# GSByeon/multi-speaker-tacotron-tensorflow

Hardware: AMD Instinct MI355X
Metric: mel-frames/sec (batched decode) (higher is better)
Workload: dtype f32 storage and accumulation; feed-forward GEMMs as 3-term split-bf16 MFMA (bf16x3), the attention memory layer as 6-term split-bf16 MFMA (operands split three ways: fp32-grade); recurrent / decoder mat-vecs exact fp32

## Files before the change

multi-speaker-tacotron-tensorflow_amd/csrc/taco_bigru_xcd.h:

```cpp
#pragma once
#include "taco_decoder_xcd.h"

#define GX_H 256
#define GX_BLK 16
typedef __attribute__((address_space(3))) float gx_lds_float;
__device__ __forceinline__ void gx_load_lds16(const float* gsrc, unsigned lds_dst) {
  unsigned keep;
  asm volatile("s_mov_b32 %0, m0\n\ts_mov_b32 m0, %2\n\ts_nop 0\n\tglobal_load_lds_dwordx4 %1, off\n\ts_mov_b32 m0, %0"
               : "=&s"(keep) : "v"(gsrc), "s"(lds_dst) : "memory");
}

#define GD_MEMBERS 32
#define GD_NREG 24
__host__ __device__ inline size_t gd_ring_floats(int RG) { return (size_t)2 * 2 * GX_BLK * RG * 24; }
__host__ __device__ inline size_t gd_lds_floats(int RG) { return gd_ring_floats(RG) + (size_t)4 * RG * GX_H + 64; }
__host__ __device__ constexpr size_t gd_xbuf_granules(int RG) { return (size_t)DX_NGROUP * 4 * RG * GX_H; }

template <int RG, int NT>
struct GdPoll {
  static constexpr int NI = (RG * GX_H + NT - 1) / NT;
  unsigned long long g[NI];
};
template <int RG, int NT>
__device__ __forceinline__ void gd_request(const dx_gu64* X, int tid, GdPoll<RG, NT>& p) {
// ... 326 lines not shown
    xs[i] = 0.f;
  }
  constexpr int QPG = UPM / 4, NIT = 2 * GX_BLK * 3 * QPG, NLD = (NIT + NT - 1) / NT;
  static_assert(NIT % 64 == 0, "a wave's 64 items are all inside the block or all outside");
  const unsigned xq_lds = (unsigned)(size_t)(gx_lds_float*)xq;
  auto blk_fetch = [&](int s0, int ring) {
#pragma unroll
    for (int u = 0; u < NLD; ++u) {
      if (u * NT + wave * 64 < NIT) {
        const int i = u * NT + tid;
        const int c = i % QPG, g = (i / QPG) % 3, j = (i / (3 * QPG)) % GX_BLK, d = i / (3 * QPG * GX_BLK);
        const int sx = min(s0 + j, T - 1);
        const float* src = a.xproj + ((size_t)row * T + sx) * 6 * H + d * 3 * H + g * H + member * UPM + 4 * c;
        const unsigned dst = __builtin_amdgcn_readfirstlane(xq_lds + (unsigned)(ring * SLOT + 4 * (u * NT + wave * 64)) * 4u);
        gx_load_lds16(src, dst);
      }
    }
  };
  blk_fetch(0, 0);
  blk_fetch(GX_BLK, 1);
  asm volatile("s_waitcnt vmcnt(0)" ::: "memory");
  __syncthreads();

  const int ui_outer = lane / LPU;
  float x0[2][3], hv[2], gv[2];
#pragma unroll
  for (int d = 0; d < 2; ++d) { hv[d] = hs[d * H + member * UPM + wave * UPW + ui_outer]; gv[d] = 0.f; }
  unsigned long long pre = 0ull, pre2 = 0ull;

  const int tid_outer = tid, lane_outer = lane;
  for (int s = 0; s < T; ++s) {
    const unsigned tag = (unsigned)s + 1u;
    int tid = tid_outer, lane = lane_outer;
    asm volatile("" : "+v"(tid), "+v"(lane));
    const int ui = lane / LPU, unit = member * UPM + wave * UPW + ui;
    const bool pub = (lane & (LPU - 1)) == 0;
    const bool active = s < L;
    GO_STAMP(0);
    const int sb = s & (GX_BLK - 1), ring = (s / GX_BLK) & 1;
    if (sb == 0 && s > 0) blk_fetch(s + GX_BLK, ring ^ 1);
    auto request = [&](const dx_gu64* Xv, int D) {
      if ((wave >> 2) == D) pre = __hip_atomic_load(Xv + (tid & 255), __ATOMIC_RELAXED, __HIP_MEMORY_SCOPE_AGENT);
    };
    auto request2 = [&](const dx_gu64* Xv, int D) {
      if ((wave >> 2) == D) pre2 = __hip_atomic_load(Xv + (tid & 255), __ATOMIC_RELAXED, __HIP_MEMORY_SCOPE_AGENT);
    };
    int csite = 0;
    auto collect = [&](const dx_gu64* Xv, unsigned tg, float* dst, int D) {
      if ((wave >> 2) == D) {
        float v[1];
        if ((unsigned)(pre2 >> 32) == tg) v[0] = __uint_as_float((unsigned)pre2);
        else if ((unsigned)(pre >> 32) == tg) v[0] = __uint_as_float((unsigned)pre);
        else { go_knob_sleep(GO_KNOB(8 + csite)); dx_poll<1>(Xv + (tid & 255), 0, tg, v, rt); }
        dst[tid & 255] = v[0];
      }
    };
    auto gates = [&](auto Dc, const dx_gu64* Xn, int Dn) {
      constexpr int D = decltype(Dc)::value;
      constexpr int R0 = (NREG / 2) * D;
#pragma unroll
      for (int g = 0; g < 3; ++g) x0[D][g] = xq[(size_t)ring * SLOT + ((size_t)(D * GX_BLK + sb) * 3 + g) * UPM + wave * UPW + ui];
      const float4 hx = *reinterpret_cast<const float4*>(hs + D * H + 4 * lane);
      taco_f32x2 acc[UPW];
#pragma unroll
      for (int i = 0; i < UPW; ++i) acc[i] = (taco_f32x2){W[R0 + 8 * i] * hx.x, W[R0 + 8 * i + 4] * hx.x};
#pragma unroll
      for (int i = 0; i < UPW; ++i) acc[i] = __builtin_elementwise_fma((taco_f32x2){hx.y, hx.y}, (taco_f32x2){W[R0 + 8 * i + 1], W[R0 + 8 * i + 5]}, acc[i]);
#pragma unroll
      for (int i = 0; i < UPW; ++i) acc[i] = __builtin_elementwise_fma((taco_f32x2){hx.z, hx.z}, (taco_f32x2){W[R0 + 8 * i + 2], W[R0 + 8 * i + 6]}, acc[i]);
#pragma unroll
      for (int i = 0; i < UPW; ++i) acc[i] = __builtin_elementwise_fma((taco_f32x2){hx.w, hx.w}, (taco_f32x2){W[R0 + 8 * i + 3], W[R0 + 8 * i + 7]}, acc[i]);
      if (GO_REQ2 && Xn && GO_KNOB(D) == 0) request2(Xn, Dn);
      else if (GO_KNOB(D) == 2) pre2 = 0ull;
      float v[2 * UPW], sm[2];
#pragma unroll
      for (int i = 0; i < UPW; ++i) { v[2 * i] = acc[i].x; v[2 * i + 1] = acc[i].y; }
      go_reduce<UPW, 2>(v, sm);
      if (GO_REQ2 && Xn && GO_KNOB(D) == 1) request2(Xn, Dn);
      const float rr = dx_sigmoid_fast(sm[0] + x0[D][0]);
      gv[D] = dx_sigmoid_fast(sm[1] + x0[D][1]);
      float rh = rr * hv[D];
      asm volatile("" : "+v"(pre), "+v"(pre2), "+v"(rh));
      if (pub) { if (GO_DYN) dx_publish(X + (size_t)D * 2 * H + unit, rh, tag, rt); else go_publish<WT>(X + (size_t)D * 2 * H + unit, rh, tag); }
      if (TAPE && pub && active) {
        float* gs = a.gsave + ((size_t)row * T + (D ? L - 1 - s : s)) * 6 * H + D * 3 * H + unit;
        gs[0] = rr; gs[H] = gv[D];
      }
    };
    auto cand = [&](auto Dc, const dx_gu64* Xn, int Dn) {
      constexpr int D = decltype(Dc)::value;
      constexpr int R0 = (NREG / 2) * D + 8 * UPW;
      const float4 hx = *reinterpret_cast<const float4*>(xs + D * H + 4 * lane);
      float v[UPW], sm[1];
      if constexpr (UPW >= 2) {
        taco_f32x2 acc[UPW / 2];
#pragma unroll
        for (int i = 0; i < UPW / 2; ++i) acc[i] = (taco_f32x2){W[R0 + 8 * i] * hx.x, W[R0 + 8 * i + 4] * hx.x};
#pragma unroll
        for (int i = 0; i < UPW / 2; ++i) acc[i] = __builtin_elementwise_fma((taco_f32x2){hx.y, hx.y}, (taco_f32x2){W[R0 + 8 * i + 1], W[R0 + 8 * i + 5]}, acc[i]);
#pragma unroll
        for (int i = 0; i < UPW / 2; ++i) acc[i] = __builtin_elementwise_fma((taco_f32x2){hx.z, hx.z}, (taco_f32x2){W[R0 + 8 * i + 2], W[R0 + 8 * i + 6]}, acc[i]);
#pragma unroll
        for (int i = 0; i < UPW / 2; ++i) acc[i] = __builtin_elementwise_fma((taco_f32x2){hx.w, hx.w}, (taco_f32x2){W[R0 + 8 * i + 3], W[R0 + 8 * i + 7]}, acc[i]);
#pragma unroll
        for (int i = 0; i < UPW / 2; ++i) { v[2 * i] = acc[i].x; v[2 * i + 1] = acc[i].y; }
      } else {
        taco_f32x2 acc = (taco_f32x2){W[R0] * hx.x, W[R0 + 1] * hx.y};
        acc = __builtin_elementwise_fma((taco_f32x2){hx.z, hx.w}, (taco_f32x2){W[R0 + 2], W[R0 + 3]}, acc);
        v[0] = acc.x + acc.y;
      }
      if (GO_REQ2 && Xn && GO_KNOB(2 + D) == 0) request2(Xn, Dn);
      else if (GO_KNOB(2 + D) == 2) pre2 = 0ull;
      go_reduce<UPW, 1>(v, sm);
      if (GO_REQ2 && Xn && GO_KNOB(2 + D) == 1) request2(Xn, Dn);
      const float cc = taco_tanh_fast(sm[0] + x0[D][2]);
      float blend = gv[D] * hv[D] + (1.f - gv[D]) * cc;
      DX_PIN(blend);
      float nv = active ? blend : hv[D];
      asm volatile("" : "+v"(pre), "+v"(pre2), "+v"(nv));
      if (pub) {
        if (GO_DYN) dx_publish(X + (size_t)(D * 2 + 1) * H + unit, nv, tag, rt); else go_publish<WT>(X + (size_t)(D * 2 + 1) * H + unit, nv, tag);
        const int t = (D && active) ? (L - 1 - s) : s;
        a.out[((size_t)row * T + t) * 2 * H + D * H + unit] = active ? nv : 0.f;
        if (TAPE && active) a.gsave[((size_t)row * T + t) * 6 * H + D * 3 * H + 2 * H + unit] = cc;
      }
      hv[D] = nv;
    };
    using F = std::integral_constant<int, 0>;
    using Bk = std::integral_constant<int, 1>;
    const dx_gu64* X_rhF = X;                  const dx_gu64* X_hF = X + (size_t)H;
    const dx_gu64* X_rhB = X + (size_t)2 * H;  const dx_gu64* X_hB = X + (size_t)3 * H;
    gates(F{}, s > 0 ? X_hB : nullptr, 1);
    GO_STAMP(1);
    csite = 0;
    if (s > 0) collect(X_hB, tag - 1u, hs + H, 1);
    __syncthreads();
    GO_STAMP(2);
    go_knob_sleep(GO_KNOB(4 + 1));
    request(X_rhF, 0);
    gates(Bk{}, X_rhF, 0);
    GO_STAMP(3);
    csite = 1;
    collect(X_rhF, tag, xs, 0);
    __syncthreads();
    GO_STAMP(4);
    go_knob_sleep(GO_KNOB(4 + 2));
    request(X_rhB, 1);
    cand(F{}, X_rhB, 1);
    GO_STAMP(5);
    csite = 2;
    collect(X_rhB, tag, xs + H, 1);
    __syncthreads();
    GO_STAMP(6);
    go_knob_sleep(GO_KNOB(4 + 3));
    request(X_hF, 0);
    cand(Bk{}, X_hF, 0);
    GO_STAMP(7);
    csite = 3;
    collect(X_hF, tag, hs, 0);
    if (sb == GX_BLK - 1) asm volatile("s_waitcnt vmcnt(0)" ::: "memory");
    __syncthreads();
    GO_STAMP(8);
    go_knob_sleep(GO_KNOB(4 + 0));
    request(X_hB, 1);
  }
}
// ... 485 lines not shown
```

multi-speaker-tacotron-tensorflow_amd/csrc/taco_decoder_xcd.h:

```cpp
#pragma once
#include "taco_kernels.h"

typedef __attribute__((address_space(1))) unsigned long long dx_gu64;
typedef __attribute__((address_space(1))) unsigned dx_gu32;

#define DX_NT 512
#define DX_NW 8
#define DX_GROUP 32
#define DX_NGROUP 8
#define DX_W 256
#define DX_P2 128
#define DX_P3 64
#define DX_SPIN_LIMIT (1u << 21)
#ifndef DX_POLL_SLEEP
#define DX_POLL_SLEEP 0
#endif
#ifndef DX_FIRST_POLL_DELAY
#define DX_FIRST_POLL_DELAY 5
#endif
#ifndef DX_PRIO_OLD
#define DX_PRIO_OLD 1
#endif
#ifndef DX_POLL_DELAY_B
#define DX_POLL_DELAY_B 5
// ... 266 lines not shown
  for (int r0 = 0; r0 < RG; r0 += 4) {
    if constexpr (RG >= 4) asm volatile("" : "+v"(xv[r0]), "+v"(xv[r0 + 1]), "+v"(xv[r0 + 2]), "+v"(xv[r0 + 3]));
    else if constexpr (RG == 2) asm volatile("" : "+v"(xv[0]), "+v"(xv[1]));
  }
}
#define DXQ_FMA(acc, xs, wp) \
  do { if (DX_DIET) acc = __builtin_elementwise_fma((taco_f32x2){xs, xs}, wp, acc); else { acc.x = fmaf((wp).x, xs, acc.x); acc.y = fmaf((wp).y, xs, acc.y); } } while (0)
template <int RG>
__device__ __forceinline__ void dxq_zero(taco_f32x2 (&acc)[RG]) {
#pragma unroll
  for (int r = 0; r < RG; ++r) acc[r] = (taco_f32x2){0.f, 0.f};
}
template <int REG0, int RG, int LD = DXS_LD>
__device__ __forceinline__ void dxw_single(const taco_f32x2 (&WP)[DX_NWP], const float* x, int lane, float (&acc)[1][RG]) {
  constexpr int k = REG0 / 2;
  dx_f32x4 xr[RG];
  dx_rows4<RG, LD>(x, lane, xr);
#pragma unroll
  for (int r = 0; r < RG; ++r) {
    const dx_f32x4 xv = xr[r];
    acc[0][r] = fmaf(WP[k].x, xv.x, acc[0][r]); acc[0][r] = fmaf(WP[k].y, xv.y, acc[0][r]);
    acc[0][r] = fmaf(WP[k + 1].x, xv.z, acc[0][r]); acc[0][r] = fmaf(WP[k + 1].y, xv.w, acc[0][r]);
  }
}
template <int REG0, int RG, int LD = DXS_LD>
__device__ __forceinline__ void dxw_pair(const taco_f32x2 (&WP)[DX_NWP], const float* x, int lane, taco_f32x2 (&acc)[RG]) {
  constexpr int k = REG0 / 2;
  dx_f32x4 xr[RG];
  dx_rows4<RG, LD>(x, lane, xr);
#pragma unroll
  for (int r = 0; r < RG; ++r) {
    const dx_f32x4 xv = xr[r];
    DXQ_FMA(acc[r], xv.x, WP[k]); DXQ_FMA(acc[r], xv.y, WP[k + 1]); DXQ_FMA(acc[r], xv.z, WP[k + 2]); DXQ_FMA(acc[r], xv.w, WP[k + 3]);
  }
}
template <int REG0, int RG, int LD = DXS_LD>
__device__ __forceinline__ void dxw_quad(const taco_f32x2 (&WP)[DX_NWP], const float* x, int lane, taco_f32x2 (&p0)[RG], taco_f32x2 (&p1)[RG]) {
  constexpr int k = REG0 / 2;
  dx_f32x4 xr[RG];
  dx_rows4<RG, LD>(x, lane, xr);
#pragma unroll
  for (int r = 0; r < RG; ++r) {
    const dx_f32x4 xv = xr[r];
    DXQ_FMA(p0[r], xv.x, WP[k]); DXQ_FMA(p1[r], xv.x, WP[k + 4]);
    DXQ_FMA(p0[r], xv.y, WP[k + 1]); DXQ_FMA(p1[r], xv.y, WP[k + 5]);
    DXQ_FMA(p0[r], xv.z, WP[k + 2]); DXQ_FMA(p1[r], xv.z, WP[k + 6]);
    DXQ_FMA(p0[r], xv.w, WP[k + 3]); DXQ_FMA(p1[r], xv.w, WP[k + 7]);
  }
}
template <int REGP, int REGS, int RG, int LD = DXS_LD>
__device__ __forceinline__ void dxw_pair_single(const taco_f32x2 (&WP)[DX_NWP], const float* x, int lane, taco_f32x2 (&p)[RG], float (&sg)[1][RG]) {
  constexpr int k = REGP / 2, ks = REGS / 2;
  dx_f32x4 xr[RG];
  dx_rows4<RG, LD>(x, lane, xr);
#pragma unroll
  for (int r = 0; r < RG; ++r) {
    const dx_f32x4 xv = xr[r];
    DXQ_FMA(p[r], xv.x, WP[k]); sg[0][r] = fmaf(WP[ks].x, xv.x, sg[0][r]);
    DXQ_FMA(p[r], xv.y, WP[k + 1]); sg[0][r] = fmaf(WP[ks].y, xv.y, sg[0][r]);
    DXQ_FMA(p[r], xv.z, WP[k + 2]); sg[0][r] = fmaf(WP[ks + 1].x, xv.z, sg[0][r]);
    DXQ_FMA(p[r], xv.w, WP[k + 3]); sg[0][r] = fmaf(WP[ks + 1].y, xv.w, sg[0][r]);
  }
}
template <int RG>
__device__ __forceinline__ void dxw_agx2(const taco_f32x2 (&WP)[DX_NWP], const float* x, int lane, taco_f32x2 (&p)[RG], float (&sg)[1][RG]) {
  constexpr int k = DXR_AGX / 2;
#pragma unroll
  for (int r = 0; r < RG; ++r) {
    const float2 xv = *reinterpret_cast<const float2*>(x + r * DXS_LD + 2 * lane);
    DXQ_FMA(p[r], xv.x, WP[k]); sg[0][r] = fmaf(WP[k + 2].x, xv.x, sg[0][r]);
    DXQ_FMA(p[r], xv.y, WP[k + 1]); sg[0][r] = fmaf(WP[k + 2].y, xv.y, sg[0][r]);
  }
}
template <int RG>
__device__ __forceinline__ void dxw_agx1(const taco_f32x2 (&WP)[DX_NWP], const float* x, int lane, taco_f32x2 (&p)[RG], float (&sg)[1][RG]) {
  constexpr int k = DXR_AGX / 2;
#pragma unroll
  for (int r = 0; r < RG; ++r) {
    const float xv = x[r * DXS_LD + lane];
    DXQ_FMA(p[r], xv, WP[k]); sg[0][r] = fmaf(WP[k + 1].x, xv, sg[0][r]);
  }
}
template <int RG>
__device__ __forceinline__ void dxw_p3(const taco_f32x2 (&WP)[DX_NWP], const float* x, int lane, float (&acc)[1][RG]) {
  constexpr int k = DXR_AGX / 2;
#pragma unroll
  for (int r = 0; r < RG; ++r) {
    const float2 xv = *reinterpret_cast<const float2*>(x + r * DXS_LD + 2 * lane);
    acc[0][r] = fmaf(WP[k + 1].y, xv.x, acc[0][r]); acc[0][r] = fmaf(WP[k + 2].x, xv.y, acc[0][r]);
  }
}
template <int RG>
__device__ __forceinline__ int dxs_row(int lane, int q) {
  if (!DX_DIET) return dx_row<RG>(lane & 3, q);
  if (RG >= 8) return ((lane >> 4) & 1) * (RG / 4) + (lane >> 5) * (RG / 2) + q;
  if (RG == 4) return lane >> 4;
  if (RG == 2) return lane >> 5;
  return 0;
}
template <int RG>
__device__ __forceinline__ bool dxs_epl(int lane) {
  if (!DX_DIET) return lane < (RG >= 4 ? 4 : RG);
  return RG >= 4 ? (lane & 15) == 0 : RG == 2 ? (lane & 31) == 0 : lane == 0;
}
template <int NC, int RG>
__device__ __forceinline__ void dxs_reduce(const float (&a)[NC][RG], float (&out)[NC][DxRL<RG>::value], int lane) {
  if constexpr (!DX_DIET) { dx_reduce<NC, RG>(a, out, lane); return; }
  else {
    constexpr int RL = DxRL<RG>::value;
    float d[NC][RL];
    if constexpr (RG >= 4) {
      constexpr int Hh = RG / 2, Q = RG / 4;
      float b[NC][Hh];
#pragma unroll
      for (int c = 0; c < NC; ++c)
#pragma unroll
        for (int p = 0; p < Hh; ++p) {
          auto r = __builtin_amdgcn_permlane32_swap(__float_as_uint(a[c][p]), __float_as_uint(a[c][Hh + p]), false, false);
          b[c][p] = __uint_as_float(r[0]) + __uint_as_float(r[1]);
        }
#pragma unroll
      for (int c = 0; c < NC; ++c)
#pragma unroll
        for (int q = 0; q < Q; ++q) {
          auto r = __builtin_amdgcn_permlane16_swap(__float_as_uint(b[c][q]), __float_as_uint(b[c][Q + q]), false, false);
          d[c][q] = __uint_as_float(r[0]) + __uint_as_float(r[1]);
        }
    } else if constexpr (RG == 2) {
#pragma unroll
      for (int c = 0; c < NC; ++c) {
        auto r = __builtin_amdgcn_permlane32_swap(__float_as_uint(a[c][0]), __float_as_uint(a[c][1]), false, false);
        d[c][0] = dx_xrow16(__uint_as_float(r[0]) + __uint_as_float(r[1]));
      }
    } else {
#pragma unroll
      for (int c = 0; c < NC; ++c) d[c][0] = dx_xrow16(dx_xrow32(a[c][0]));
    }
#pragma unroll
    for (int c = 0; c < NC; ++c)
#pragma unroll
      for (int q = 0; q < RL; ++q) d[c][q] += DX_DPP0(d[c][q], 0xB1);
#pragma unroll
    for (int c = 0; c < NC; ++c)
#pragma unroll
      for (int q = 0; q < RL; ++q) d[c][q] += DX_DPP0(d[c][q], 0x4E);
#pragma unroll
    for (int c = 0; c < NC; ++c)
#pragma unroll
      for (int q = 0; q < RL; ++q) d[c][q] += DX_DPP0(d[c][q], 0x141);
#pragma unroll
    for (int c = 0; c < NC; ++c)
#pragma unroll
      for (int q = 0; q < RL; ++q) {
        out[c][q] = d[c][q] + DX_DPP0(d[c][q], 0x140);
        asm("" : "+v"(out[c][q]));
      }
  }
}

#ifndef DX_DLY_TUNED
#define DX_DLY_TUNED 1
#endif
__host__ __device__ constexpr int dx_site_delay(int site, int dflt, int RG = 4) {
  constexpr int tuned4[11] = {4, 5, 6, 5, 0, 0, 5, 5, 0, 4, 0};
  constexpr int tuned8[11] = {7, 5, 3, 5, 0, 6, 5, 6, 4, 6, 2};
  return DX_DLY_TUNED ? (RG == 8 ? tuned8[site] : tuned4[site]) : dflt;
}
#ifdef DX_DLY_RT
__constant__ int g_dx_dly[32];
#define DX_DLY(site, dflt) (100 + (site))
#else
#define DX_DLY(site, dflt) dx_site_delay(site, dflt, RG)
#endif
struct DxRt {
  dx_gu32* err; bool wt; bool dead;
#ifdef DX_DLY_RT
  int dly[12];
#endif
};
template <int DLY>
__device__ __forceinline__ void dx_first_poll_sleep(const DxRt& rt) {
#ifdef DX_DLY_RT
  if constexpr (DLY >= 100) { const int n = __builtin_amdgcn_readfirstlane(rt.dly[DLY - 100]); for (int i = 0; i < n; ++i) __builtin_amdgcn_s_sleep(1); return; }
#endif
  if constexpr (DLY > 0 && DLY < 100) __builtin_amdgcn_s_sleep(DLY);
  (void)rt;
}
#ifndef DX_PUB_MODE
#define DX_PUB_MODE 0
#endif
__device__ __forceinline__ void dx_store_local(dx_gu64* p, unsigned long long g) {
  if (DX_PUB_MODE == 1) (void)__hip_atomic_exchange(p, g, __ATOMIC_RELAXED, __HIP_MEMORY_SCOPE_WORKGROUP);
  else if (DX_PUB_MODE == 2) __builtin_nontemporal_store(g, p);
  else if (DX_PUB_MODE == 3) *p = g;
  else __hip_atomic_store(p, g, __ATOMIC_RELAXED, __HIP_MEMORY_SCOPE_WORKGROUP);
}
__device__ __forceinline__ dx_gu64* dx_at(const dx_gu64* X, unsigned idx) {
  return (dx_gu64*)((__attribute__((address_space(1))) char*)X + (size_t)(idx * 8u));
}
template <int WTC = -1>
__device__ __forceinline__ void dx_publish(dx_gu64* p, float v, unsigned tag, const DxRt& rt) {
  const unsigned long long g = ((unsigned long long)tag << 32) | (unsigned long long)__float_as_uint(v);
  if (WTC == 1 || (WTC < 0 && rt.wt)) __hip_atomic_store(p, g, __ATOMIC_RELAXED, __HIP_MEMORY_SCOPE_AGENT);
  else dx_store_local(p, g);
}
template <int N, int WTC = -1>
__device__ __forceinline__ void dx_publish_n(dx_gu64* p, int stride, const float (&v)[N], unsigned tag, const DxRt& rt) {
  unsigned long long g[N];
#pragma unroll
  for (int u = 0; u < N; ++u) g[u] = ((unsigned long long)tag << 32) | (unsigned long long)__float_as_uint(v[u]);
  if (WTC == 1 || (WTC < 0 && rt.wt)) {
#pragma unroll
    for (int u = 0; u < N; ++u) __hip_atomic_store(p + u * stride, g[u], __ATOMIC_RELAXED, __HIP_MEMORY_SCOPE_AGENT);
  } else {
#pragma unroll
    for (int u = 0; u < N; ++u) dx_store_local(p + u * stride, g[u]);
  }
}
#define DX_PIN(x) asm("" : "+v"(x))
template <int N, int DLY = 0>
__device__ __forceinline__ void dx_poll_at(const dx_gu64* X, unsigned idx0, unsigned stride, unsigned tag, float (&v)[N], DxRt& rt) {
  unsigned long long g[N];
  unsigned spins = 0;
  dx_first_poll_sleep<DLY>(rt);
  for (;;) {
    bool ok = true;
#pragma unroll
    for (int u = 0; u < N; ++u) g[u] = __hip_atomic_load(dx_at(X, idx0 + (unsigned)u * stride), __ATOMIC_RELAXED, __HIP_MEMORY_SCOPE_AGENT);
#pragma unroll
    for (int u = 0; u < N; ++u) ok = ok && ((unsigned)(g[u] >> 32) == tag);
    if (ok || rt.dead) break;
    if (DX_POLL_SLEEP) __builtin_amdgcn_s_sleep(DX_POLL_SLEEP);
    if ((++spins & 1023u) == 0) {
      if (spins >= DX_SPIN_LIMIT || __hip_atomic_load(rt.err, __ATOMIC_RELAXED, __HIP_MEMORY_SCOPE_AGENT) != 0) {
        __hip_atomic_store(rt.err, 2u, __ATOMIC_RELAXED, __HIP_MEMORY_SCOPE_AGENT);
        rt.dead = true;
      }
    }
  }
#pragma unroll
  for (int u = 0; u < N; ++u) v[u] = __uint_as_float((unsigned)g[u]);
}
template <int N, int DLY = 0>
__device__ __forceinline__ void dx_poll(const dx_gu64* p0, size_t stride, unsigned tag, float (&v)[N], DxRt& rt) {
  dx_poll_at<N, DLY>(p0, 0u, (unsigned)stride, tag, v, rt);
}
typedef unsigned long long dx_u64x2 __attribute__((ext_vector_type(2)));
// ... 244 lines not shown
  const int NCF = (a.rM + DX_GROUP - 1) / DX_GROUP;

  for (int i = tid; i < TS * (DS / 4); i += DX_NT) {
    const int j = i / (DS / 4), d4 = i % (DS / 4);
    float4 k4 = make_float4(0.f, 0.f, 0.f, 0.f);
    if (brow < a.B && j < psn) k4 = *reinterpret_cast<const float4*>(a.keys + ((size_t)brow * T + ps0 + j) * AW + cb * DS + 4 * d4);
    *reinterpret_cast<float4*>(Kc + (size_t)j * DS + 4 * d4) = k4;
  }
  for (int i = tid; i < T * (DC / 4); i += DX_NT) {
    const int j = i / (DC / 4), d4 = i % (DC / 4);
    float4 v4 = make_float4(0.f, 0.f, 0.f, 0.f);
    if (brow < a.B) v4 = *reinterpret_cast<const float4*>(a.values + ((size_t)brow * T + j) * DX_W + asl * DC + 4 * d4);
    *reinterpret_cast<float4*>(Vc + (size_t)j * DC + 4 * d4) = v4;
  }
  for (int i = tid; i < RG * DXS_LD; i += DX_NT) st[i] = 0.f;
  __syncthreads();
  for (int i = tid; i < RG * DX_W; i += DX_NT) {
    const int r = i / DX_W, nn = i % DX_W, b = row0 + r;
    if (b < a.B) {
      if (a.h_att0) st[r * DXS_LD + DXS_HATT + nn] = a.h_att0[(size_t)b * DX_W + nn];
      if (a.h10) st[r * DXS_LD + DXS_H1 + nn] = a.h10[(size_t)b * DX_W + nn];
      if (a.h20) st[r * DXS_LD + DXS_H2 + nn] = a.h20[(size_t)b * DX_W + nn];
    }
    st[r * DXS_LD + DXS_T + nn] = fmaxf(a.b_p1_0[nn], 0.f);
  }
  for (int j = tid; j < Tpad; j += DX_NT) { alp[j] = (a.att_type == 2 && j == 0) ? 1.f : 0.f; sc[j] = 0.f; tmp[j] = 0.f; tmp2[j] = 0.f; }
  if (tid < DS) { vv[tid] = a.att_v[cb * DS + tid]; bq[tid] = a.att_b ? a.att_b[cb * DS + tid] : 0.f; qv[tid] = 0.f; }
  if (tid < DXB_N * DX_NW) {
    const int e = tid / DX_NW, w = tid % DX_NW, n8 = member * 8 + w;
    float v = 0.f;
    switch (e) {
      case DXB_P1: v = (TAPE && a.p1o_raw) ? a.b_p1_0[n8] : a.b_p1c[n8]; break;
      case DXB_P2: if (w < 4) v = a.b_p2[member * 4 + w]; break;
      case DXB_AR: v = a.b_ag[n8]; break;
      case DXB_AU: v = a.b_ag[DX_W + n8]; break;
      case DXB_AC: v = a.b_ac[n8]; break;
      case DXB_G1R: v = a.b_g1f[n8]; break;
      case DXB_G1U: v = a.b_g1f[DX_W + n8]; break;
      case DXB_G1X: v = a.b_g1f[2 * DX_W + n8]; break;
      case DXB_O0: v = a.b_g1f[3 * DX_W + n8]; break;
      case DXB_G1C: v = a.b_g1c[n8]; break;
      case DXB_G2R: v = a.b_g2g[n8]; break;
      case DXB_G2U: v = a.b_g2g[DX_W + n8]; break;
      case DXB_G2C: v = a.b_g2c[n8]; break;
      case DXB_F0: if (w < NCF && member * NCF + w < a.rM) v = a.b_f[member * NCF + w]; break;
      case DXB_F1: if (w + 8 < NCF && member * NCF + w + 8 < a.rM) v = a.b_f[member * NCF + w + 8]; break;
      case DXB_P3: if (PD == 3 && w < 2) v = a.b_p3[member * 2 + w]; break;
      default: break;
    }
    bl[tid] = v;
  }
  for (int i = tid; i < DXRB_N * RG * DX_NW; i += DX_NT) {
    const int e = i / (RG * DX_NW), r = (i / DX_NW) % RG, w = i % DX_NW, b = row0 + r, n8 = member * 8 + w;
    float v = 0.f;
    switch (e) {
      case DXRB_AR: v = a.b_ag[n8]; break;
      case DXRB_AU: v = a.b_ag[DX_W + n8]; break;
      case DXRB_AX: v = 0.f; break;
      case DXRB_G1R: v = a.b_g1f[n8]; break;
      case DXRB_G1U: v = a.b_g1f[DX_W + n8]; break;
      case DXRB_G1X: v = a.b_g1f[2 * DX_W + n8]; break;
      default: v = a.b_g1f[3 * DX_W + n8]; break;
    }
    if (a.rowbias && b < a.B) v += a.rowbias[((size_t)b * DXRB_N + e) * DX_W + n8];
    rbl[i] = v;
  }
  const float sbias = (a.att_type == 2 && a.score_bias) ? a.score_bias[0] : 0.f;
  constexpr bool man = MAN;
  const unsigned mrow_lds = (unsigned)(size_t)(dx_lds_float*)mrow;
  const unsigned tfb_lds = (unsigned)(size_t)(dx_lds_float*)tfb;
  if (TAPE) for (int i = tid; i < RG * DX_W; i += DX_NT) tfb[i] = 0.f;
  __syncthreads();

  constexpr int RL = DxRL<RG>::value;
  const bool epl = dxs_epl<RG>(lane);
  const int en = member * 8 + wave;
  int erow[RL];
#pragma unroll
  for (int q = 0; q < RL; ++q) erow[q] = dxs_row<RG>(lane, q);
#define DX_RB(slot, q) rbl[((slot) * RG + erow[q]) * DX_NW + wave]
#define DX_BIAS_AHEAD(var, slot) float var = bl[(slot) * DX_NW + wave]
#define DX_BIAS_HERE(var) asm volatile("" : "+v"(var))
  float g_u[RL], g_cx[RL], g_h[RL], g_o0[RL];
  unsigned trow[RL];
  bool tval[RL];
  float g_o1[RL];
  const unsigned tstr = (unsigned)a.tstride;
#pragma unroll
  for (int q = 0; q < RL; ++q) {
    trow[q] = (unsigned)(row0 + erow[q]) * (unsigned)a.n * DX_W + (unsigned)en;
    tval[q] = TAPE && a.tape && epl && (row0 + erow[q] < a.B);
    g_o1[q] = 0.f;
  }
#define DX_TAPE(slot, q, val) do { if (TAPE && tval[q]) a.tape[(unsigned)(slot) * tstr + trow[q] + (unsigned)t * DX_W] = (val); } while (0)
  if (TAPE) {
    const int t = 0;
#pragma unroll
    for (int q = 0; q < RL; ++q) DX_TAPE(DXT_P1, q, fmaxf(a.b_p1_0[en], 0.f));
  }

  if (DX_PRIO_OLD && wave < 4) __builtin_amdgcn_s_setprio(DX_PRIO_OLD);
  const int tid_outer = tid, lane_outer = lane;
  for (int t = 0; t < a.n; ++t) {
    const unsigned tag = (unsigned)t + 1u;
    int tid = tid_outer, lane = lane_outer;
    asm volatile("" : "+v"(tid), "+v"(lane));
    int erow[RL];
#pragma unroll
    for (int q = 0; q < RL; ++q) erow[q] = dxs_row<RG>(lane, q);
    DX_STAMP(0);
    if (man) {
      const float* src = a.manual + ((size_t)min(brow, a.B - 1) * a.n + t) * T;
      for (int j0 = wave * 64; j0 < T; j0 += DX_NT)
        dx_load_lds4(src + min(j0 + lane, T - 1), __builtin_amdgcn_readfirstlane(mrow_lds + (unsigned)j0 * 4u));
    }
    if (TAPE && a.teacher && wave < RG && t + 1 < a.n) {
      const float* src = a.teacher + ((size_t)min(row0 + wave, a.B - 1) * a.n + t) * a.mels;
      for (int j0 = 0; j0 < a.mels; j0 += 64)
        dx_load_lds4(src + min(j0 + lane, a.mels - 1), __builtin_amdgcn_readfirstlane(tfb_lds + (unsigned)(wave * DX_W + j0) * 4u));
    }
    if (wave < 4) {
      float acc[1][RG], s[1][RL];
      DX_BIAS_AHEAD(b_p2, DXB_P2);
      dx_zero<1, RG>(acc);
      dxw_single<DXR_P2, RG>(WP, st + DXS_T, lane, acc);
      DX_BIAS_HERE(b_p2);
      dxs_reduce<1, RG>(acc, s, lane);
      if (epl) {
#pragma unroll
        for (int q = 0; q < RL; ++q) {
          const float p2v = fmaxf(s[0][q] + b_p2, 0.f);
          dx_publish<WTC>(dx_at(X, (unsigned)(xl.p2 + erow[q] * DX_P2 + member * 4 + wave)), p2v, tag, rt);
          if (TAPE && tval[q] && a.tp_p2) a.tp_p2[((size_t)(row0 + erow[q]) * a.n + t) * a.ld_p2 + member * 4 + wave] = p2v;
        }
      }
    }
#pragma unroll
    for (int q = 0; q < RL; ++q) g_h[q] = st[erow[q] * DXS_LD + DXS_HATT + en];
    taco_f32x2 ag01[RG];
    float ag2[1][RG];
    dxq_zero<RG>(ag01);
    dx_zero<1, RG>(ag2);
    dxw_pair<DXR_AGH, RG>(WP, st + DXS_HATT, lane, ag01);
    dx_ahead<RG>(ag01);
    dx_gather_at<RG, DX_P2, false, DXS_LD, DX_NT, DX_DLY(0, DX_POLL_DELAY_B)>(X, (unsigned)xl.p2, tag, st, DXS_P2, 0, 0, tid, rt);
    __syncthreads();
    if constexpr (PD == 3) {
      if (wave < 2) {
        float acc[1][RG], s[1][RL];
        dx_zero<1, RG>(acc);
        dxw_p3<RG>(WP, st + DXS_P2, lane, acc);
        dxs_reduce<1, RG>(acc, s, lane);
        if (epl) {
#pragma unroll
          for (int q = 0; q < RL; ++q)
            dx_publish<WTC>(dx_at(X, (unsigned)(xl.p3 + erow[q] * DX_P3 + member * 2 + wave)), fmaxf(s[0][q] + bl[DXB_P3 * DX_NW + wave], 0.f), tag, rt);
        }
      }
      dx_gather_at<RG, DX_P3, false, DXS_LD, DX_NT, DX_DLY(1, DX_FIRST_POLL_DELAY)>(X, (unsigned)xl.p3, tag, st, DXS_OUT2, 0, 0, tid, rt);
      __syncthreads();
    }
    DX_STAMP(1);
    {
      float s[3][RL];
      if constexpr (PD == 3) dxw_agx1<RG>(WP, st + DXS_OUT2, lane, ag01, ag2);
      else dxw_agx2<RG>(WP, st + DXS_P2, lane, ag01, ag2);
      float aga[3][RG];
#pragma unroll
      for (int r = 0; r < RG; ++r) { aga[0][r] = ag01[r].x; aga[1][r] = ag01[r].y; aga[2][r] = ag2[0][r]; }
      dxs_reduce<3, RG>(aga, s, lane);
#pragma unroll
      for (int q = 0; q < RL; ++q) {
        const float rg = dx_sigmoid_fast(s[0][q] + DX_RB(DXRB_AR, q));
        g_u[q] = dx_sigmoid_fast(s[1][q] + DX_RB(DXRB_AU, q));
        g_cx[q] = s[2][q] + DX_RB(DXRB_AX, q);
        if (epl) dx_publish<WTC>(dx_at(X, (unsigned)(xl.rha + erow[q] * DX_W + en)), rg * g_h[q], tag, rt);
        DX_TAPE(DXT_RA, q, rg); DX_TAPE(DXT_UA, q, g_u[q]); DX_TAPE(DXT_RHA, q, rg * g_h[q]);
      }
    }
    DX_BIAS_AHEAD(b_ac, DXB_AC);
    dx_gather_at<RG, DX_W, false, DXS_LD, DX_NT, DX_DLY(2, DX_FIRST_POLL_DELAY)>(X, (unsigned)xl.rha, tag, st, DXS_T, 0, 0, tid, rt);
    DX_BIAS_HERE(b_ac);
    __syncthreads();
    DX_STAMP(2);
    {
      float acc[1][RG], s[1][RL];
      dx_zero<1, RG>(acc);
      dxw_single<DXR_AC, RG>(WP, st + DXS_T, lane, acc);
      dxs_reduce<1, RG>(acc, s, lane);
#pragma unroll
      for (int q = 0; q < RL; ++q) {
        const float c = taco_tanh_fast(g_cx[q] + s[0][q] + b_ac);
        const float hn = g_u[q] * g_h[q] + (1.f - g_u[q]) * c;
        if (epl) dx_publish<WTC>(dx_at(X, (unsigned)(xl.ha + erow[q] * DX_W + en)), hn, tag, rt);
        DX_TAPE(DXT_CA, q, c); DX_TAPE(DXT_HA, q, hn);
      }
    }
#pragma unroll
    for (int q = 0; q < RL; ++q) g_h[q] = st[erow[q] * DXS_LD + DXS_H1 + en];
    dx_gather_at<RG, DX_W, false, DXS_LD, DX_NT, DX_DLY(3, DX_FIRST_POLL_DELAY)>(X, (unsigned)xl.ha, tag, st, DXS_HATT, 0, 0, tid, rt);
    __syncthreads();
    DX_STAMP(3);
    if (!man) {
      {
        const float4 xv = *reinterpret_cast<const float4*>(st + arow * DXS_LD + DXS_HATT + 4 * lane);
        float qa[QC][1], qs[QC][1];
        static_assert(QC % 2 == 0, "query columns in pairs");
#pragma unroll
        for (int i = 0; i < QC; i += 2) {
          taco_f32x2 q2 = {0.f, 0.f};
          DXQ_FMA(q2, xv.x, WQP[2 * i + 0]); DXQ_FMA(q2, xv.y, WQP[2 * i + 1]); DXQ_FMA(q2, xv.z, WQP[2 * i + 2]); DXQ_FMA(q2, xv.w, WQP[2 * i + 3]);
          qa[i][0] = q2.x; qa[i + 1][0] = q2.y;
        }
        dxs_reduce<QC, 1>(qa, qs, lane);
        float qme = qs[0][0];
#pragma unroll
        for (int i = 1; i < QC; ++i) qme = (lane >= i) ? qs[i][0] : qme;
        if (lane < QC) qv[wave * QC + lane] = qme + bq[wave * QC + lane];
        if (TAPE && a.tape && lane < QC && pb == 0 && brow < a.B)
          a.tape[(unsigned)DXT_Q * tstr + ((unsigned)brow * (unsigned)a.n + (unsigned)t) * DX_W + cb * DS + wave * QC + lane] = qme;
      }
      __syncthreads();
      DX_STAMP(4);
      {
        const int jl = lane >> 2, cp = lane & 3;
        constexpr bool QV_REG = CH < 16;
        float qreg[QV_REG ? CH : 1], vreg[QV_REG ? CH : 1];
        if constexpr (QV_REG) {
#pragma unroll
          for (int c = 0; c < CH; ++c) { qreg[c] = qv[cp * CH + c]; vreg[c] = vv[cp * CH + c]; }
        }
        for (int j0 = 0; j0 < psn; j0 += 16 * DX_NW) {
          const int j = j0 + wave * 16 + jl;
          const int jc = j < psn ? j : psn - 1;
          const float* kp = Kc + (size_t)jc * DS + cp * CH;
          float e = 0.f;
#pragma unroll
          for (int c = 0; c < CH; c += 4) {
            const float4 k4 = *reinterpret_cast<const float4*>(kp + c);
            if constexpr (QV_REG) {
              e += vreg[c] * taco_tanh_fast(k4.x + qreg[c]) + vreg[c + 1] * taco_tanh_fast(k4.y + qreg[c + 1]) +
                   vreg[c + 2] * taco_tanh_fast(k4.z + qreg[c + 2]) + vreg[c + 3] * taco_tanh_fast(k4.w + qreg[c + 3]);
            } else {
              const float4 q4 = *reinterpret_cast<const float4*>(qv + cp * CH + c), v4 = *reinterpret_cast<const float4*>(vv + cp * CH + c);
              e += v4.x * taco_tanh_fast(k4.x + q4.x) + v4.y * taco_tanh_fast(k4.y + q4.y) +
                   v4.z * taco_tanh_fast(k4.z + q4.z) + v4.w * taco_tanh_fast(k4.w + q4.w);
// ... 3 lines not shown
          if (cp == 0 && j < psn) dx_publish<WTC>(dx_at(X, (unsigned)(xl.sc + (arow * Pc + cb) * T + ps0 + j)), e, tag, rt);
        }
      }
    }
    constexpr bool G1_AHEAD = RG < 8;
    taco_f32x2 g1p0[RG], g1p1[RG];
    dxq_zero<RG>(g1p0); dxq_zero<RG>(g1p1);
    if (G1_AHEAD) {
      dxw_pair<DXR_G1H, RG>(WP, st + DXS_H1, lane, g1p0);
      dxw_quad<DXR_G1A, RG>(WP, st + DXS_HATT, lane, g1p0, g1p1);
      dx_ahead<RG>(g1p0); dx_ahead<RG>(g1p1);
    }
    int aoff = 0;
    if (!man) {
      {
        const int jl = lane >> 2, part = lane & 3;
        for (int j0 = 0; j0 < T; j0 += 16 * DX_NW) {
          const int j = j0 + wave * 16 + jl;
          float s = 0.f;
          if (j < T) {
            float v[NP];
            dx_poll_at<NP, DX_DLY(4, DX_POLL_DELAY_B)>(X, (unsigned)(xl.sc + (arow * Pc + part * NP) * T + j), (unsigned)T, tag, v, rt);
#pragma unroll
            for (int u = 0; u < NP; ++u) s += v[u];
          }
          s = dx_quadsum(s);
          if (part == 0 && j < T) sc[j] = s;
        }
      }
      __syncthreads();
      DX_STAMP(5);
      if (TAPE && a.tp_e && tid < TP && asl * TP + tid < T && brow < a.B)
        a.tp_e[((size_t)brow * a.n + t) * T + asl * TP + tid] = sc[asl * TP + tid];
      if (TAPE) __syncthreads();
      if (wave == 0) {
        const int C = (T + 63) >> 6;
        const int j0 = lane * C;
        if (C <= 2) dx_normalise<2>(sc, alp, j0, min(C, max(T - j0, 0)), a.att_type, sbias);
        else if (C <= 8) dx_normalise<8>(sc, alp, j0, min(C, max(T - j0, 0)), a.att_type, sbias);
        else dx_normalise_lds(sc, tmp, tmp2, alp, j0, min(j0 + C, T), a.att_type, sbias);
      }
      __syncthreads();
    } else {
      asm volatile("s_waitcnt vmcnt(0)" ::: "memory");
      __syncthreads();
      aoff = (int)(mrow - sc);
    }
    {
      constexpr int JL = 64 / DC;
      const int d = lane % DC, jsub = lane / DC;
      float part = 0.f;
      for (int j = wave * JL + jsub; j < T; j += DX_NW * JL) part = fmaf(sc[aoff + j], Vc[(size_t)j * DC + d], part);
      if (DC <= 32) part = dx_xrow32(part);
      if (DC <= 16) part = dx_xrow16(part);
      if (DC <= 8) part += DX_DPP0(part, 0x128);
      if (lane < DC) cpart[wave * 64 + lane] = part;
    }
    __syncthreads();
    if (tid < DC) {
      float s = 0.f;
#pragma unroll
      for (int w = 0; w < DX_NW; ++w) s += cpart[w * 64 + tid];
      dx_publish<WTC>(dx_at(X, (unsigned)(xl.ctx + arow * DX_W + asl * DC + tid)), s, tag, rt);
      if (TAPE && a.tp_ctx && brow < a.B) a.tp_ctx[((size_t)brow * a.n + t) * a.ld_ctx + asl * DC + tid] = s;
    }
    {
      for (int j = tid; j < T; j += DX_NT) alp[j] = sc[aoff + j];
      const int p0 = asl * TP;
      if (tid < TP && p0 + tid < T && brow < a.B) {
        if (a.hist) a.hist[((size_t)brow * T + p0 + tid) * a.n + t] = sc[aoff + p0 + tid];
        if (TAPE && a.tp_alpha) a.tp_alpha[((size_t)brow * (a.n + 1) + t + 1) * T + p0 + tid] = sc[aoff + p0 + tid];
      }
    }
    dx_gather_at<RG, DX_W, false, DXS_LD, DX_NT, DX_DLY(5, DX_FIRST_POLL_DELAY)>(X, (unsigned)xl.ctx, tag, st, DXS_CTX, 0, 0, tid, rt);
    __syncthreads();
    DX_STAMP(6);
    {
      float s[4][RL];
      if (!G1_AHEAD) {
        dxq_zero<RG>(g1p0); dxq_zero<RG>(g1p1);
        dxw_pair<DXR_G1H, RG>(WP, st + DXS_H1, lane, g1p0);
        dxw_quad<DXR_G1A, RG>(WP, st + DXS_HATT, lane, g1p0, g1p1);
      }
      dxw_quad<DXR_G1B, RG>(WP, st + DXS_CTX, lane, g1p0, g1p1);
      float g1a[4][RG];
#pragma unroll
      for (int r = 0; r < RG; ++r) { g1a[0][r] = g1p0[r].x; g1a[1][r] = g1p0[r].y; g1a[2][r] = g1p1[r].x; g1a[3][r] = g1p1[r].y; }
      dxs_reduce<4, RG>(g1a, s, lane);
      DX_STAMP(12);
#pragma unroll
      for (int q = 0; q < RL; ++q) {
        const float rg = dx_sigmoid_fast(s[0][q] + DX_RB(DXRB_G1R, q));
        g_u[q] = dx_sigmoid_fast(s[1][q] + DX_RB(DXRB_G1U, q));
        g_cx[q] = s[2][q] + DX_RB(DXRB_G1X, q);
        g_o0[q] = s[3][q] + DX_RB(DXRB_O0, q);
        if (epl) dx_publish<WTC>(dx_at(X, (unsigned)(xl.rh1 + erow[q] * DX_W + en)), rg * g_h[q], tag, rt);
        DX_TAPE(DXT_R1, q, rg); DX_TAPE(DXT_U1, q, g_u[q]); DX_TAPE(DXT_RH1, q, rg * g_h[q]); DX_TAPE(DXT_O0, q, g_o0[q]);
      }
      DX_STAMP(13);
    }
    DX_BIAS_AHEAD(b_g1c, DXB_G1C);
    dx_gather_at<RG, DX_W, false, DXS_LD, DX_NT, DX_DLY(6, DX_FIRST_POLL_DELAY)>(X, (unsigned)xl.rh1, tag, st, DXS_T, 0, 0, tid, rt);
    DX_BIAS_HERE(b_g1c);
    DX_STAMP(14);
    __syncthreads();
    DX_STAMP(7);
    {
      float acc[1][RG], s[1][RL];
      dx_zero<1, RG>(acc);
      dxw_single<DXR_G1C, RG>(WP, st + DXS_T, lane, acc);
      dxs_reduce<1, RG>(acc, s, lane);
#pragma unroll
      for (int q = 0; q < RL; ++q) {
        const float c = taco_tanh_fast(g_cx[q] + s[0][q] + b_g1c);
        const float hn = g_u[q] * g_h[q] + (1.f - g_u[q]) * c;
        g_o1[q] = hn + g_o0[q];
        if (epl) {
          dx_publish<WTC>(dx_at(X, (unsigned)(xl.h1 + erow[q] * DX_W + en)), hn, tag, rt);
          dx_publish<WTC>(dx_at(X, (unsigned)(xl.o1 + erow[q] * DX_W + en)), hn + g_o0[q], tag, rt);
        }
        DX_TAPE(DXT_C1, q, c); DX_TAPE(DXT_H1, q, hn); DX_TAPE(DXT_O1, q, g_o1[q]);
      }
    }
#pragma unroll
    for (int q = 0; q < RL; ++q) g_h[q] = st[erow[q] * DXS_LD + DXS_H2 + en];
    taco_f32x2 g2p[RG];
    float g2c[1][RG];
    dxq_zero<RG>(g2p);
    dx_zero<1, RG>(g2c);
    if (G1_AHEAD) { dxw_pair<DXR_G2H, RG>(WP, st + DXS_H2, lane, g2p); dx_ahead<RG>(g2p); }
    dx_gather_at<RG, DX_W, false, DXS_LD, DX_NT, DX_DLY(7, DX_POLL_DELAY_B)>(X, (unsigned)xl.h1, tag, st, DXS_H1, 0, 0, tid, rt);
    dx_gather_at<RG, DX_W, false, DXS_LD, DX_NT, 0>(X, (unsigned)xl.o1, tag, st, DXS_OUT1, 0, 0, tid, rt);
    __syncthreads();
    DX_STAMP(8);
    {
      float s[3][RL];
      if (!G1_AHEAD) dxw_pair<DXR_G2H, RG>(WP, st + DXS_H2, lane, g2p);
      dxw_pair_single<DXR_G2X, DXR_G2X + 8, RG>(WP, st + DXS_OUT1, lane, g2p, g2c);
      float g2a[3][RG];
#pragma unroll
      for (int r = 0; r < RG; ++r) { g2a[0][r] = g2p[r].x; g2a[1][r] = g2p[r].y; g2a[2][r] = g2c[0][r]; }
      dxs_reduce<3, RG>(g2a, s, lane);
#pragma unroll
      for (int q = 0; q < RL; ++q) {
        const float rg = dx_sigmoid_fast(s[0][q] + bl[DXB_G2R * DX_NW + wave]);
        g_u[q] = dx_sigmoid_fast(s[1][q] + bl[DXB_G2U * DX_NW + wave]);
        g_cx[q] = s[2][q];
        if (epl) dx_publish<WTC>(dx_at(X, (unsigned)(xl.rh2 + erow[q] * DX_W + en)), rg * g_h[q], tag, rt);
        DX_TAPE(DXT_R2, q, rg); DX_TAPE(DXT_U2, q, g_u[q]); DX_TAPE(DXT_RH2, q, rg * g_h[q]);
      }
    }
    DX_BIAS_AHEAD(b_g2c, DXB_G2C);
    dx_gather_at<RG, DX_W, false, DXS_LD, DX_NT, DX_DLY(8, DX_FIRST_POLL_DELAY)>(X, (unsigned)xl.rh2, tag, st, DXS_T, 0, 0, tid, rt);
    DX_BIAS_HERE(b_g2c);
    __syncthreads();
    DX_STAMP(9);
    {
      float acc[1][RG], s[1][RL];
      dx_zero<1, RG>(acc);
      dxw_single<DXR_G2C, RG>(WP, st + DXS_T, lane, acc);
      dxs_reduce<1, RG>(acc, s, lane);
#pragma unroll
      for (int q = 0; q < RL; ++q) {
        const float c = taco_tanh_fast(g_cx[q] + s[0][q] + b_g2c);
        const float hn = g_u[q] * g_h[q] + (1.f - g_u[q]) * c;
        if (epl) dx_publish<WTC>(dx_at(X, (unsigned)(xl.h2 + erow[q] * DX_W + en)), hn, tag, rt);
        DX_TAPE(DXT_C2, q, c); DX_TAPE(DXT_H2, q, hn); DX_TAPE(DXT_O2, q, hn + g_o1[q]);
      }
    }
    float p1a[1][RG];
    dx_zero<1, RG>(p1a);
    if (G1_AHEAD) { dxw_single<DXR_P1C, RG>(WP, st + DXS_CTX, lane, p1a); dx_ahead<RG>(p1a); }
    DX_BIAS_AHEAD(b_p1, DXB_P1); DX_BIAS_AHEAD(b_f0, DXB_F0); DX_BIAS_AHEAD(b_f1, DXB_F1);
    dx_gather_at<RG, DX_W, true, DXS_LD, DX_NT, DX_DLY(9, DX_POLL_DELAY_B)>(X, (unsigned)xl.h2, tag, st, DXS_H2, DXS_OUT1, DXS_OUT2, tid, rt);
    DX_BIAS_HERE(b_p1); DX_BIAS_HERE(b_f0); DX_BIAS_HERE(b_f1);
    __syncthreads();
    DX_STAMP(10);
    auto store_frame = [&](int q, float y0, float y1, bool share) {
      const int b = row0 + erow[q];
      const int n0 = member * NCF + wave, n1 = n0 + 8;
      const bool v0 = wave < NCF && n0 < a.rM, v1 = wave + 8 < NCF && n1 < a.rM;
      if (b < a.B) {
        float* mrow = a.mel + (size_t)b * a.n * a.rM + (size_t)t * a.rM;
        bool nzf = false;
        if (v0) { mrow[n0] = y0; nzf = nzf || (y0 != 0.f); }
        if (v1) { mrow[n1] = y1; nzf = nzf || (y1 != 0.f); }
        if (nzf) a.nz[(size_t)t * a.B + b] = 1;
      }
      if (share) {
        const int f0 = a.rM - a.mels;
        if (v0 && n0 >= f0) dx_publish<WTC>(dx_at(X, (unsigned)(xl.fb + erow[q] * DX_P2 + (n0 - f0))), y0, tag, rt);
        if (v1 && n1 >= f0) dx_publish<WTC>(dx_at(X, (unsigned)(xl.fb + erow[q] * DX_P2 + (n1 - f0))), y1, tag, rt);
      }
    };
    if (TAPE && a.own_fb) {
      {
        taco_f32x2 fp[RG];
        float fa[2][RG], s[2][RL];
        dxq_zero<RG>(fp);
        dxw_pair<DXR_F, RG>(WP, st + DXS_OUT2, lane, fp);
#pragma unroll
        for (int r = 0; r < RG; ++r) { fa[0][r] = fp[r].x; fa[1][r] = fp[r].y; }
        dxs_reduce<2, RG>(fa, s, lane);
        if (epl) {
#pragma unroll
          for (int q = 0; q < RL; ++q) store_frame(q, s[0][q] + bl[DXB_F0 * DX_NW + wave], s[1][q] + bl[DXB_F1 * DX_NW + wave], t + 1 < a.n);
        }
      }
      if (t + 1 < a.n) {
        for (int i = tid; i < RG * a.mels; i += DX_NT) {
          const int r = i / a.mels, j = i - r * a.mels;
          float v[1];
          dx_poll_at<1>(X, (unsigned)(xl.fb + r * DX_P2 + j), 0u, tag, v, rt);
          tfb[r * DX_W + j] = v[0];
        }
      }
      __syncthreads();
      {
        float pa[1][RG], s[1][RL];
#pragma unroll
        for (int r = 0; r < RG; ++r) pa[0][r] = p1a[0][r];
        if (!G1_AHEAD) dxw_single<DXR_P1C, RG>(WP, st + DXS_CTX, lane, pa);
        dxw_single<DXR_P1O, RG, DX_W>(WP, tfb, lane, pa);
        dxs_reduce<1, RG>(pa, s, lane);
        if (epl && t + 1 < a.n) {
#pragma unroll
          for (int q = 0; q < RL; ++q) {
            const float p1v = fmaxf(s[0][q] + bl[DXB_P1 * DX_NW + wave], 0.f);
            dx_publish<WTC>(dx_at(X, (unsigned)(xl.p1 + erow[q] * DX_W + en)), p1v, tag, rt);
            if (tval[q]) a.tape[(unsigned)DXT_P1 * tstr + trow[q] + (unsigned)(t + 1) * DX_W] = p1v;
          }
        }
// ... 55 lines not shown
```

Before: 6.433 million.

## Publish GRU reset-gate product before computing update and candidate gates

```diff
diff --git a/multi-speaker-tacotron-tensorflow_amd/csrc/taco_bigru_xcd.h b/multi-speaker-tacotron-tensorflow_amd/csrc/taco_bigru_xcd.h
--- a/multi-speaker-tacotron-tensorflow_amd/csrc/taco_bigru_xcd.h
+++ b/multi-speaker-tacotron-tensorflow_amd/csrc/taco_bigru_xcd.h
@@ -432,6 +432,7 @@
       float rh = rr * hv[D];
       asm volatile("" : "+v"(pre), "+v"(pre2), "+v"(rh));
       if (pub) { if (GO_DYN) dx_publish(X + (size_t)D * 2 * H + unit, rh, tag, rt); else go_publish<WT>(X + (size_t)D * 2 * H + unit, rh, tag); }
+      GO_STAMP(9 + D);
       if (TAPE && pub && active) {
         float* gs = a.gsave + ((size_t)row * T + (D ? L - 1 - s : s)) * 6 * H + D * 3 * H + unit;
         gs[0] = rr; gs[H] = gv[D];
diff --git a/multi-speaker-tacotron-tensorflow_amd/csrc/taco_decoder_xcd.h b/multi-speaker-tacotron-tensorflow_amd/csrc/taco_decoder_xcd.h
--- a/multi-speaker-tacotron-tensorflow_amd/csrc/taco_decoder_xcd.h
+++ b/multi-speaker-tacotron-tensorflow_amd/csrc/taco_decoder_xcd.h
@@ -372,6 +372,40 @@
   }
 }
 template <int RG>
+__device__ __forceinline__ void dxw_agx2_pair(const taco_f32x2 (&WP)[DX_NWP], const float* x, int lane, taco_f32x2 (&p)[RG]) {
+  constexpr int k = DXR_AGX / 2;
+#pragma unroll
+  for (int r = 0; r < RG; ++r) {
+    const float2 xv = *reinterpret_cast<const float2*>(x + r * DXS_LD + 2 * lane);
+    DXQ_FMA(p[r], xv.x, WP[k]); DXQ_FMA(p[r], xv.y, WP[k + 1]);
+  }
+}
+template <int RG>
+__device__ __forceinline__ void dxw_agx2_single(const taco_f32x2 (&WP)[DX_NWP], const float* x, int lane, float (&sg)[1][RG]) {
+  constexpr int k = DXR_AGX / 2;
+#pragma unroll
+  for (int r = 0; r < RG; ++r) {
+    const float2 xv = *reinterpret_cast<const float2*>(x + r * DXS_LD + 2 * lane);
+    sg[0][r] = fmaf(WP[k + 2].x, xv.x, sg[0][r]); sg[0][r] = fmaf(WP[k + 2].y, xv.y, sg[0][r]);
+  }
+}
+template <int RG>
+__device__ __forceinline__ void dxw_agx1_pair(const taco_f32x2 (&WP)[DX_NWP], const float* x, int lane, taco_f32x2 (&p)[RG]) {
+  constexpr int k = DXR_AGX / 2;
+#pragma unroll
+  for (int r = 0; r < RG; ++r) DXQ_FMA(p[r], x[r * DXS_LD + lane], WP[k]);
+}
+template <int RG>
+__device__ __forceinline__ void dxw_agx1_single(const taco_f32x2 (&WP)[DX_NWP], const float* x, int lane, float (&sg)[1][RG]) {
+  constexpr int k = DXR_AGX / 2;
+#pragma unroll
+  for (int r = 0; r < RG; ++r) sg[0][r] = fmaf(WP[k + 1].x, x[r * DXS_LD + lane], sg[0][r]);
+}
+#ifndef DX_PUB_FIRST
+#define DX_PUB_FIRST 7
+#endif
+__device__ __forceinline__ void dx_behind_publish() { asm volatile("" ::: "memory"); }
+template <int RG>
 __device__ __forceinline__ void dxw_p3(const taco_f32x2 (&WP)[DX_NWP], const float* x, int lane, float (&acc)[1][RG]) {
   constexpr int k = DXR_AGX / 2;
 #pragma unroll
@@ -452,7 +486,7 @@
 #define DX_DLY_TUNED 1
 #endif
 __host__ __device__ constexpr int dx_site_delay(int site, int dflt, int RG = 4) {
-  constexpr int tuned4[11] = {4, 5, 6, 5, 0, 0, 5, 5, 0, 4, 0};
+  constexpr int tuned4[11] = {2, 5, 0, 5, 0, 3, 2, 3, 0, 3, 0};
   constexpr int tuned8[11] = {7, 5, 3, 5, 0, 6, 5, 6, 4, 6, 2};
   return DX_DLY_TUNED ? (RG == 8 ? tuned8[site] : tuned4[site]) : dflt;
 }
@@ -863,6 +897,7 @@
 #define DX_BIAS_AHEAD(var, slot) float var = bl[(slot) * DX_NW + wave]
 #define DX_BIAS_HERE(var) asm volatile("" : "+v"(var))
   float g_u[RL], g_cx[RL], g_h[RL], g_o0[RL];
+  constexpr bool PF_A = (DX_PUB_FIRST & 1) && RG < 8, PF_1 = (DX_PUB_FIRST & 2) && RG < 8, PF_2 = (DX_PUB_FIRST & 4) && RG < 8;
   unsigned trow[RL];
   bool tval[RL];
   float g_o1[RL];
@@ -942,7 +977,32 @@
       __syncthreads();
     }
     DX_STAMP(1);
-    {
+    if constexpr (PF_A) {
+      float ar[1][RG], sr[1][RL], rgv[RL];
+      if constexpr (PD == 3) dxw_agx1_pair<RG>(WP, st + DXS_OUT2, lane, ag01);
+      else dxw_agx2_pair<RG>(WP, st + DXS_P2, lane, ag01);
+#pragma unroll
+      for (int r = 0; r < RG; ++r) ar[0][r] = ag01[r].x;
+      dxs_reduce<1, RG>(ar, sr, lane);
+#pragma unroll
+      for (int q = 0; q < RL; ++q) {
+        rgv[q] = dx_sigmoid_fast(sr[0][q] + DX_RB(DXRB_AR, q));
+        if (epl) dx_publish<WTC>(dx_at(X, (unsigned)(xl.rha + erow[q] * DX_W + en)), rgv[q] * g_h[q], tag, rt);
+      }
+      dx_behind_publish();
+      float au[2][RG], su[2][RL];
+      if constexpr (PD == 3) dxw_agx1_single<RG>(WP, st + DXS_OUT2, lane, ag2);
+      else dxw_agx2_single<RG>(WP, st + DXS_P2, lane, ag2);
+#pragma unroll
+      for (int r = 0; r < RG; ++r) { au[0][r] = ag01[r].y; au[1][r] = ag2[0][r]; }
+      dxs_reduce<2, RG>(au, su, lane);
+#pragma unroll
+      for (int q = 0; q < RL; ++q) {
+        g_u[q] = dx_sigmoid_fast(su[0][q] + DX_RB(DXRB_AU, q));
+        g_cx[q] = su[1][q] + DX_RB(DXRB_AX, q);
+        DX_TAPE(DXT_RA, q, rgv[q]); DX_TAPE(DXT_UA, q, g_u[q]); DX_TAPE(DXT_RHA, q, rgv[q] * g_h[q]);
+      }
+    } else {
       float s[3][RL];
       if constexpr (PD == 3) dxw_agx1<RG>(WP, st + DXS_OUT2, lane, ag01, ag2);
       else dxw_agx2<RG>(WP, st + DXS_P2, lane, ag01, ag2);
@@ -1112,6 +1172,33 @@
         dxw_pair<DXR_G1H, RG>(WP, st + DXS_H1, lane, g1p0);
         dxw_quad<DXR_G1A, RG>(WP, st + DXS_HATT, lane, g1p0, g1p1);
       }
+      if constexpr (PF_1) {
+        float ar[1][RG], sr[1][RL], rgv[RL];
+        dxw_pair<DXR_G1B, RG>(WP, st + DXS_CTX, lane, g1p0);
+#pragma unroll
+        for (int r = 0; r < RG; ++r) ar[0][r] = g1p0[r].x;
+        dxs_reduce<1, RG>(ar, sr, lane);
+        DX_STAMP(12);
+#pragma unroll
+        for (int q = 0; q < RL; ++q) {
+          rgv[q] = dx_sigmoid_fast(sr[0][q] + DX_RB(DXRB_G1R, q));
+          if (epl) dx_publish<WTC>(dx_at(X, (unsigned)(xl.rh1 + erow[q] * DX_W + en)), rgv[q] * g_h[q], tag, rt);
+        }
+        DX_STAMP(13);
+        dx_behind_publish();
+        dxw_pair<DXR_G1B + 8, RG>(WP, st + DXS_CTX, lane, g1p1);
+        float g1d[3][RG], sd[3][RL];
+#pragma unroll
+        for (int r = 0; r < RG; ++r) { g1d[0][r] = g1p0[r].y; g1d[1][r] = g1p1[r].x; g1d[2][r] = g1p1[r].y; }
+        dxs_reduce<3, RG>(g1d, sd, lane);
+#pragma unroll
+        for (int q = 0; q < RL; ++q) {
+          g_u[q] = dx_sigmoid_fast(sd[0][q] + DX_RB(DXRB_G1U, q));
+          g_cx[q] = sd[1][q] + DX_RB(DXRB_G1X, q);
+          g_o0[q] = sd[2][q] + DX_RB(DXRB_O0, q);
+          DX_TAPE(DXT_R1, q, rgv[q]); DX_TAPE(DXT_U1, q, g_u[q]); DX_TAPE(DXT_RH1, q, rgv[q] * g_h[q]); DX_TAPE(DXT_O0, q, g_o0[q]);
+        }
+      } else {
       dxw_quad<DXR_G1B, RG>(WP, st + DXS_CTX, lane, g1p0, g1p1);
       float g1a[4][RG];
 #pragma unroll
@@ -1128,6 +1215,7 @@
         DX_TAPE(DXT_R1, q, rg); DX_TAPE(DXT_U1, q, g_u[q]); DX_TAPE(DXT_RH1, q, rg * g_h[q]); DX_TAPE(DXT_O0, q, g_o0[q]);
       }
       DX_STAMP(13);
+      }
     }
     DX_BIAS_AHEAD(b_g1c, DXB_G1C);
     dx_gather_at<RG, DX_W, false, DXS_LD, DX_NT, DX_DLY(6, DX_FIRST_POLL_DELAY)>(X, (unsigned)xl.rh1, tag, st, DXS_T, 0, 0, tid, rt);
@@ -1166,6 +1254,30 @@
     {
       float s[3][RL];
       if (!G1_AHEAD) dxw_pair<DXR_G2H, RG>(WP, st + DXS_H2, lane, g2p);
+      if constexpr (PF_2) {
+        float ar[1][RG], sr[1][RL], rgv[RL];
+        dxw_pair<DXR_G2X, RG>(WP, st + DXS_OUT1, lane, g2p);
+#pragma unroll
+        for (int r = 0; r < RG; ++r) ar[0][r] = g2p[r].x;
+        dxs_reduce<1, RG>(ar, sr, lane);
+#pragma unroll
+        for (int q = 0; q < RL; ++q) {
+          rgv[q] = dx_sigmoid_fast(sr[0][q] + bl[DXB_G2R * DX_NW + wave]);
+          if (epl) dx_publish<WTC>(dx_at(X, (unsigned)(xl.rh2 + erow[q] * DX_W + en)), rgv[q] * g_h[q], tag, rt);
+        }
+        dx_behind_publish();
+        dxw_single<DXR_G2X + 8, RG>(WP, st + DXS_OUT1, lane, g2c);
+        float g2d[2][RG], sd[2][RL];
+#pragma unroll
+        for (int r = 0; r < RG; ++r) { g2d[0][r] = g2p[r].y; g2d[1][r] = g2c[0][r]; }
+        dxs_reduce<2, RG>(g2d, sd, lane);
+#pragma unroll
+        for (int q = 0; q < RL; ++q) {
+          g_u[q] = dx_sigmoid_fast(sd[0][q] + bl[DXB_G2U * DX_NW + wave]);
+          g_cx[q] = sd[1][q];
+          DX_TAPE(DXT_R2, q, rgv[q]); DX_TAPE(DXT_U2, q, g_u[q]); DX_TAPE(DXT_RH2, q, rgv[q] * g_h[q]);
+        }
+      } else {
       dxw_pair_single<DXR_G2X, DXR_G2X + 8, RG>(WP, st + DXS_OUT1, lane, g2p, g2c);
       float g2a[3][RG];
 #pragma unroll
@@ -1178,6 +1290,7 @@
         g_cx[q] = s[2][q];
         if (epl) dx_publish<WTC>(dx_at(X, (unsigned)(xl.rh2 + erow[q] * DX_W + en)), rg * g_h[q], tag, rt);
         DX_TAPE(DXT_R2, q, rg); DX_TAPE(DXT_U2, q, g_u[q]); DX_TAPE(DXT_RH2, q, rg * g_h[q]);
+      }
       }
     }
     DX_BIAS_AHEAD(b_g2c, DXB_G2C);
```

New measurement: 6.523 million (median of 6 runs). 1.01x the previous value.
